# unibas-gravis/icp-proposal

Measured on AMD Instinct MI355X. Metric: ICP-proposal MH iterations/sec (femur GPMM r=50, ~50k-vtx target), higher is better.
Workload: dtype f64

## Files before the change

__graft_entry__.py:

```python
from __future__ import annotations

import importlib.util
import os
import subprocess
import sys

ROOT = os.path.dirname(os.path.abspath(__file__))
PKG_DIR = os.path.join(ROOT, "icp-proposal_amd")


def load_package():
    if "icp_proposal_amd" in sys.modules:
        return sys.modules["icp_proposal_amd"]
    spec = importlib.util.spec_from_file_location("icp_proposal_amd", os.path.join(PKG_DIR, "__init__.py"),
                                                  submodule_search_locations=[PKG_DIR])
    mod = importlib.util.module_from_spec(spec)
    sys.modules["icp_proposal_amd"] = mod
    spec.loader.exec_module(mod)
    return mod


def build() -> None:
    subprocess.run(["make", "-C", os.path.join(PKG_DIR, "csrc"), "-j4"], check=True)
    host_mk = os.path.join(PKG_DIR, "host", "Makefile")
    if os.path.exists(host_mk):
        subprocess.run(["make", "-C", os.path.join(PKG_DIR, "host")], check=True)
    subprocess.run(["make", "-C", os.path.join(ROOT, "oracle")], check=True)
    subprocess.run(["make", "-C", os.path.join(ROOT, "tests", "support")], check=True)
    pkg = load_package()
    pkg._native.lib()


def smoke() -> None:
    import numpy as np

    pkg = load_package()
    sys.path.insert(0, ROOT)
    from oracle import oracle as O

    model, target = pkg.data.load_femur_model_and_target(50)
    ctx = pkg.IcpContext(model, target, device=0)
    om, ot = O.OracleModel.from_model(model), O.OracleMesh(target.points, target.cells)
    r = model.rank
    rng = np.random.default_rng(7)
    theta = pkg.initial_parameters(model)
    theta[10:] = 0.3 * rng.normal(size=r)
    z = rng.normal(size=r)
    tp = pkg.data.decimated_point_subset(target, 2 * r)
    for direction, pp in ((pkg.ModelSampling, O.proposal_params(0.1, 10.0, 5.0, O.MODEL_SAMPLING, True, n_model_ids=2 * r)),
                          (pkg.TargetSampling, O.proposal_params(0.1, 10.0, 5.0, O.TARGET_SAMPLING, True, target_pts=tp))):
        prop = pkg.NonRigidIcpProposal(ctx, 0.1, 10.0, 5.0, 2 * r, direction, True, decimatedTargetPoints=tp)
        got, corr = prop.propose(theta, z, return_correspondences=True)
        want = O.propose(om, ot, pp, theta, z)
        post = O.icp_posterior(om, ot, pp, theta)
        assert np.array_equal(corr, np.where(post.keep == 1, post.corr_id, -1)), "correspondence indices differ"
        rel = np.abs(got - want).max() / np.abs(want[10:]).max()
        assert rel < 1e-5, f"proposed coefficients differ: {rel}"
        lt, lo = prop.logTransitionProbability(theta, got), O.log_transition(om, ot, pp, theta, want)
        assert abs(lt - lo) <= 1e-5 * abs(lo), (lt, lo)
        prop.close()
    ev = pkg.IndependentPointDistanceEvaluator(ctx, 0.0, 2.0, pkg.ModelToTargetEvaluation, 4 * r, decimatedTargetPoints=tp)
    ep = O.evaluator_params(O.EVAL_INDEPENDENT, O.MODEL_TO_TARGET, n_model_ids=4 * r, target_pts=tp, p0=0.0, p1=2.0)
    lv, (lvo, _) = ev.logValue(theta), O.evaluator_log_value(om, ot, ep, theta)
    assert abs(lv - lvo) <= 1e-9 * abs(lvo), (lv, lvo)
    ev.close()
    ctx.close()
    print("smoke ok: correspondence indices bit-exact, coefficients/logT/logValue within tolerance")


if __name__ == "__main__":
    build()
    if len(sys.argv) > 1 and sys.argv[1] == "smoke":
        smoke()
```

icp-proposal_amd/csrc/kernels_eigen.hip:

```cpp
#include <algorithm>
#include <atomic>
#include <cstdio>
#include <cstdlib>

#include "icp_kernels.hpp"
#include "icp_dense.hpp"

namespace icp {

#ifdef ICP_EIGEN_TIMING
__device__ long long g_eigen_stamps[64];
#define EIG_STAMP(i) do { if (threadIdx.x == 0) g_eigen_stamps[i] = __builtin_amdgcn_s_memrealtime(); } while (0)
#else
#define EIG_STAMP(i)
#endif
}
#include "icp_tridiag.hpp"
namespace icp {

namespace {

constexpr int kEigenMaxSweeps = 40;
#ifndef ICP_LOOSE_TAU
#define ICP_LOOSE_TAU 4e-6
// ... 100 lines not shown
      const double vkp = V[op], vkq = V[oq];
      V[op] = c * vkp - s * vkq;
      V[oq] = s * vkp + c * vkq;
    }
  };
  int converged = 0, n_sweeps = 0;
  for (int sweep = 0; sweep < 40 && !converged; ++sweep) {
    for (int rnd = 0; rnd < mm; ++rnd) {
      if (tid < half) {
        const int p = ra < rb ? ra : rb, q = ra < rb ? rb : ra;
        double c = 1.0, s = 0.0;
        if (q < r) {
          const double apq = A[p * lda + q], app = A[p * lda + p], aqq = A[q * lda + q];
          if (fabs(apq) > 1e-300 && apq * apq > 1e-36 * fabs(app * aqq)) {
            const double a = 0.5 * (aqq - app);
            const double h2 = fma(a, a, apq * apq);
            const double h = h2 * fast_rsqrt(h2);
            const double t = (a >= 0.0 ? apq : -apq) * fast_rcp(fabs(a) + h);
            c = fast_rsqrt(fma(t, t, 1.0));
            s = t * c;
          }
        }
        s_p[tid] = (short)p; s_q[tid] = (short)q; s_c[tid] = c; s_s[tid] = s;
        if (tid == 0) { rb = rb + 1 == mm ? 0 : rb + 1; }
        else { ra = ra + 1 == mm ? 0 : ra + 1; rb = rb + 1 == mm ? 0 : rb + 1; }
      }
      __syncthreads();
#pragma unroll
      for (int m = 0; m < kItems; ++m) {
        if (it_a[m] >= 0) {
          if (it_a[m] & 0x40000000) do_vpair(it_a[m] & 0x3FFFFFFF, it_b[m]);
          else do_block(it_a[m], it_b[m]);
        }
      }
      for (int w = tid + nt * kItems; w < n_items; w += nt) {
        if (w < n_blocks) {
          int P1 = 0, base = 0;
          while (base + (half - P1) <= w) { base += half - P1; ++P1; }
          do_block(P1, P1 + (w - base));
        } else {
          const int vi = w - n_blocks;
          do_vpair(vi / half, vi % half);
        }
      }
      __syncthreads();
    }
    double off = 0.0, dg = 0.0;
    for (int e = tid; e < r * r; e += nt) {
      const int i = e / r, j = e - i * r;
      const double v = A[(size_t)i * lda + j];
      if (i == j) dg = fma(v, v, dg);
      else off = fma(v, v, off);
    }
    off = block_sum(off, s_red);
    dg = block_sum(dg, s_red);
    converged = off <= 1e-26 * dg;
    n_sweeps = sweep + 1;
  }
  if (tid == 0) { status[0] = converged ? 0 : 2; status[-1] = n_sweeps; }
  for (int i = tid; i < r; i += nt) s_mu[i] = A[(size_t)i * lda + i];
  __syncthreads();
  for (int i = tid; i < r; i += nt) {
    int rank = 0;
    const double mi = s_mu[i];
    for (int j = 0; j < r; ++j) rank += (s_mu[j] < mi) || (s_mu[j] == mi && j < i);
    s_rank[i] = rank;
    int best = 0;
    double bv = fabs(V[i]);
    for (int k = 1; k < r; ++k) {
      const double a = fabs(V[(size_t)k * ldv + i]);
      if (a > bv) { bv = a; best = k; }
    }
    s_sgn[i] = V[(size_t)best * ldv + i] < 0.0 ? -1.0 : 1.0;
    Sout[rank] = 1.0 / mi;
  }
  __syncthreads();
  if (!v_in_lds) {
    for (int e = tid; e < r * r; e += nt) work[e] = V[e];
    __syncthreads();
    V = work;
  }
  for (int e = tid; e < r * r; e += nt) {
    const int k = e / r, i = e - k * r;
    const double v = V[(size_t)k * ldv + i] * s_sgn[i];
    Vout[(size_t)k * r + s_rank[i]] = v;
    Vtout[(size_t)s_rank[i] * r + k] = v;
  }
}


__device__ __forceinline__ int rr_dst(int pos, int m) {
  const int k = pos >> 1;
  if ((pos & 1) == 0) return k == 0 ? 0 : (k == m - 1 ? 2 * (m - 1) + 1 : 2 * (k + 1));
  return k == 0 ? 2 : 2 * (k - 1) + 1;
}
__device__ __forceinline__ int rr_src(int pos, int m) {
  const int k = pos >> 1;
  if ((pos & 1) == 0) return k == 0 ? 0 : (k == 1 ? 1 : 2 * (k - 1));
  return k == m - 1 ? 2 * (m - 1) : 2 * (k + 1) + 1;
}

struct Rot { double c, s; };

__device__ __forceinline__ Rot jacobi_rotation(double app, double apq, double aqq) {
  const double a = aqq - app, b = apq + apq, b2 = b * b;
  const bool rot = apq * apq > 1e-36 * fabs(app * aqq);
  const double h2 = fma(a, a, b2);
  const double h = h2 * __builtin_amdgcn_rsq(h2);
  const double u = h + fabs(a);
  const double w = fma(u, u, b2);
  const double y0 = __builtin_amdgcn_rsq(w);
  const double e = fma(-(0.5 * w) * y0, y0, 0.5);
  const double y = fma(y0, e * fma(1.5, e, 1.0), y0);
  Rot R;
  R.c = rot ? u * y : 1.0;
  R.s = rot ? (a >= 0.0 ? b : -b) * y : 0.0;
  return R;
}

struct B22 { double a00, a01, a10, a11; };

__device__ __forceinline__ B22 rot_block(B22 b, double c1, double s1, double c2, double s2) {
  const double t00 = fma(c1, b.a00, -(s1 * b.a10)), t01 = fma(c1, b.a01, -(s1 * b.a11));
  const double t10 = fma(s1, b.a00, c1 * b.a10), t11 = fma(s1, b.a01, c1 * b.a11);
  return B22{fma(c2, t00, -(s2 * t01)), fma(s2, t00, c2 * t01), fma(c2, t10, -(s2 * t11)), fma(s2, t10, c2 * t11)};
}
typedef double dbl2 __attribute__((ext_vector_type(2)));
__device__ __forceinline__ dbl2 lds2(const double* p) { return *(const dbl2*)p; }


constexpr int kPwRoundsMask = 0x3FFFF, kPwAbort = 1 << 18, kPwFinished = 1 << 19, kPwIdShift = 20, kPwIdMask = 0x7FF;
__device__ __forceinline__ void progress_publish(int* meta, int id, int rounds, int flags) {
  __hip_atomic_store(meta, (id << kPwIdShift) | flags | rounds, __ATOMIC_RELAXED, __HIP_MEMORY_SCOPE_AGENT);
}

__device__ __forceinline__ double wave_shr1_f64(double v) {
  const int lo = __builtin_amdgcn_update_dpp(__double2loint(v), __double2loint(v), 0x138, 0xf, 0xf, false);
  const int hi = __builtin_amdgcn_update_dpp(__double2hiint(v), __double2hiint(v), 0x138, 0xf, 0xf, false);
  return __hiloint2double(hi, lo);
}
__device__ __forceinline__ double wave_shl1_f64(double v) {
  const int lo = __builtin_amdgcn_update_dpp(__double2loint(v), __double2loint(v), 0x130, 0xf, 0xf, false);
  const int hi = __builtin_amdgcn_update_dpp(__double2hiint(v), __double2hiint(v), 0x130, 0xf, 0xf, false);
  return __hiloint2double(hi, lo);
}

constexpr int kReplayStageRounds = 64;
constexpr int kReplayWaves = 8;
constexpr int kReplayRows = 4 * kReplayWaves;
constexpr int kEigMetaCorr = 7;
constexpr int kEigMetaMu = 64;
constexpr int kEigMetaXchg = 128;

__device__ __forceinline__ void sc1_store(double* p, double v) { __hip_atomic_store(p, v, __ATOMIC_RELAXED, __HIP_MEMORY_SCOPE_AGENT); }
__device__ __forceinline__ double sc1_load(const double* p) { return __hip_atomic_load(p, __ATOMIC_RELAXED, __HIP_MEMORY_SCOPE_AGENT); }

__device__ void eigen_replay_consumer(int r, const double* Vwarm, const double* rotlog, int* meta, const double* xcorr ,
                                      double* Vout, double* Vtout, double* Sout, int launch_id, int me, int nb, int* done_word,
                                      int done_value) {
  __shared__ int s_pw;
  const int tid = threadIdx.x, lane = tid & 63, wave = tid >> 6;
  const int n2 = (r + 1) & ~1, m = n2 >> 1;
  double* s_log = s_dyn;
  const int kc = lane >> 5, q = lane & 31, ka = kReplayRows * me + 4 * wave + 2 * kc, kb = ka + 1;
  const bool carry = wave < kReplayWaves && kReplayRows * me + 4 * wave < r;
  const bool act = q < m && carry;
  const int qc = q < m ? q : 0;
  auto v0_at = [&](int k, int p) { return (k < r && p < r) ? (Vwarm ? Vwarm[(size_t)k * r + p] : (k == p ? 1.0 : 0.0)) : 0.0; };
  double a0 = act ? v0_at(ka, 2 * q) : 0.0, a1 = act ? v0_at(ka, 2 * q + 1) : 0.0;
  double b0 = act ? v0_at(kb, 2 * q) : 0.0, b1 = act ? v0_at(kb, 2 * q + 1) : 0.0;
  int done = 0;
  bool aborted = false;
  for (;;) {
    if (tid == 0) {
      int pw;
      for (;;) {
        pw = __hip_atomic_load(meta, __ATOMIC_RELAXED, __HIP_MEMORY_SCOPE_AGENT);
        if (((pw >> kPwIdShift) & kPwIdMask) == launch_id && ((pw & kPwRoundsMask) > done || (pw & (kPwAbort | kPwFinished)))) break;
        __builtin_amdgcn_s_sleep(2);
      }
      s_pw = pw;
#ifdef ICP_EIGEN_TIMING
      if (me == 0 && (pw & kPwFinished)) g_eigen_stamps[40] = __builtin_amdgcn_s_memrealtime();
#endif
    }
    __syncthreads();
    const int pw = s_pw;
    if (pw & kPwAbort) { aborted = true; break; }
    const int avail = pw & kPwRoundsMask;
    while (done < avail) {
      const int n = min(avail - done, kReplayStageRounds);
      for (int e = tid; e < 2 * n * m; e += blockDim.x) s_log[e] = sc1_load(rotlog + 2 * (size_t)done * m + e);
      __syncthreads();
      if (carry) {
        for (int rl = 0; rl < n; rl += 8) {
          dbl2 cs[8];
#pragma unroll
          for (int u = 0; u < 8; ++u) cs[u] = *(const dbl2*)&s_log[2 * (min(rl + u, n - 1) * m + qc)];
#pragma unroll
          for (int u = 0; u < 8; ++u) {
            if (rl + u < n) {
              const double fa = fma(cs[u].x, a0, cs[u].y * a1), ga = fma(-cs[u].y, a0, cs[u].x * a1);
              const double fb = fma(cs[u].x, b0, cs[u].y * b1), gb = fma(-cs[u].y, b0, cs[u].x * b1);
              const double ua = wave_shr1_f64(q == 0 ? ga : fa), da = wave_shl1_f64(ga);
              const double ub = wave_shr1_f64(q == 0 ? gb : fb), db = wave_shl1_f64(gb);
              a0 = q == 0 ? fa : ua; a1 = q == m - 1 ? fa : da;
              b0 = q == 0 ? fb : ub; b1 = q == m - 1 ? fb : db;
            }
          }
        }
      }
      __syncthreads();
      done += n;
    }
    if (pw & kPwFinished) break;
  }
#ifdef ICP_EIGEN_TIMING
  if (me == 0 && tid == 0) g_eigen_stamps[41] = __builtin_amdgcn_s_memrealtime();
#endif
  double* s_x = s_dyn;
  double* s_mu = s_dyn + 4096;
  int* s_rank = (int*)(s_dyn + 4096 + 64);
  double* s_bv = s_dyn + 4096 + 128;
  int* s_bk = (int*)(s_dyn + 4096 + 192);
  double* s_pv = s_dyn + 4096 + 256;
  int* s_pk = (int*)(s_dyn + 4096 + 256 + kReplayWaves * 64);
  double* xchg = (double*)meta + kEigMetaXchg;
  if (!aborted) {
    const int has_corr = __hip_atomic_load(meta + kEigMetaCorr, __ATOMIC_RELAXED, __HIP_MEMORY_SCOPE_AGENT);
    if (tid < n2) s_mu[tid] = sc1_load((const double*)meta + kEigMetaMu + tid);
    if (has_corr)
      for (int e = tid; e < n2 * n2; e += blockDim.x) s_x[e] = sc1_load(xcorr + e);
    __syncthreads();
    if (has_corr) {
      if (act) {
        *(dbl2*)&s_dyn[5632 + (4 * wave + 2 * kc) * 64 + 2 * q] = dbl2{a0, a1};
        *(dbl2*)&s_dyn[5632 + (4 * wave + 2 * kc + 1) * 64 + 2 * q] = dbl2{b0, b1};
      }
      __syncthreads();
      if (carry) {
        double ca0 = 0.0, ca1 = 0.0, cb0 = 0.0, cb1 = 0.0;
        const int ra = 5632 + (4 * wave + 2 * kc) * 64, rb = ra + 64;
        for (int i = 0; i < n2; i += 2) {
          const dbl2 va = *(const dbl2*)&s_dyn[ra + i], vb = *(const dbl2*)&s_dyn[rb + i];
          const dbl2 xe = *(const dbl2*)&s_dyn[i * n2 + 2 * qc], xo = *(const dbl2*)&s_dyn[(i + 1) * n2 + 2 * qc];
          ca0 = fma(va.x, xe.x, ca0); ca1 = fma(va.x, xe.y, ca1); cb0 = fma(vb.x, xe.x, cb0); cb1 = fma(vb.x, xe.y, cb1);
          ca0 = fma(va.y, xo.x, ca0); ca1 = fma(va.y, xo.y, ca1); cb0 = fma(vb.y, xo.x, cb0); cb1 = fma(vb.y, xo.y, cb1);
        }
        if (act) { a0 += ca0; a1 += ca1; b0 += cb0; b1 += cb1; }
      }
    }
    if (wave < kReplayWaves) {
      const bool va = act && ka < r, vb = act && kb < r;
      double m0 = va ? fabs(a0) : -1.0, m1 = va ? fabs(a1) : -1.0, c0 = a0, c1 = a1;
      int k0 = ka, k1 = ka;
      if (vb && fabs(b0) > m0) { m0 = fabs(b0); c0 = b0; k0 = kb; }
      if (vb && fabs(b1) > m1) { m1 = fabs(b1); c1 = b1; k1 = kb; }
      const double o0 = __shfl_xor(m0, 32, 64), o1 = __shfl_xor(m1, 32, 64), w0 = __shfl_xor(c0, 32, 64), w1 = __shfl_xor(c1, 32, 64);
      const int ok0 = __shfl_xor(k0, 32, 64), ok1 = __shfl_xor(k1, 32, 64);
      if (o0 > m0 || (o0 == m0 && ok0 < k0)) { m0 = o0; c0 = w0; k0 = ok0; }
      if (o1 > m1 || (o1 == m1 && ok1 < k1)) { m1 = o1; c1 = w1; k1 = ok1; }
      if (lane < 32 && q < m) {
        s_pv[wave * 64 + 2 * q] = m0 < 0.0 ? 0.0 : c0; s_pk[wave * 64 + 2 * q] = m0 < 0.0 ? 0x7fffffff : k0;
        s_pv[wave * 64 + 2 * q + 1] = m1 < 0.0 ? 0.0 : c1; s_pk[wave * 64 + 2 * q + 1] = m1 < 0.0 ? 0x7fffffff : k1;
      }
    }
    __syncthreads();
    if (tid < n2) {
      double bv = s_pv[tid];
      int bk = s_pk[tid];
      for (int w = 1; w < kReplayWaves; ++w) {
        const double v = s_pv[w * 64 + tid];
        const int kk = s_pk[w * 64 + tid];
        if (kk != 0x7fffffff && (bk == 0x7fffffff || fabs(v) > fabs(bv) || (fabs(v) == fabs(bv) && kk < bk))) { bv = v; bk = kk; }
      }
      s_bv[tid] = bv; s_bk[tid] = bk;
      if (nb > 1) { sc1_store(xchg + me * 128 + tid, bv); sc1_store(xchg + me * 128 + 64 + tid, (double)bk); }
      int rank = 0;
      const double mi = s_mu[tid];
      for (int j = 0; j < n2; ++j) rank += (s_mu[j] < mi) || (s_mu[j] == mi && j < tid);
      s_rank[tid] = rank;
      if (me == 0 && rank < r) sc1_store(Sout + rank, 1.0 / mi);
    }
    if (nb > 1) {
      asm volatile("s_waitcnt vmcnt(0)" ::: "memory");
      __syncthreads();
      const int o = 1 - me;
      if (tid == 0) {
        __hip_atomic_store(meta + 2 + me, launch_id, __ATOMIC_RELAXED, __HIP_MEMORY_SCOPE_AGENT);
        while (__hip_atomic_load(meta + 2 + o, __ATOMIC_RELAXED, __HIP_MEMORY_SCOPE_AGENT) != launch_id) __builtin_amdgcn_s_sleep(1);
      }
      __syncthreads();
      if (tid < n2) {
        const double v = sc1_load(xchg + o * 128 + tid);
        const int kk = (int)sc1_load(xchg + o * 128 + 64 + tid);
        double bv = s_bv[tid];
        const int bk = s_bk[tid];
        if (kk != 0x7fffffff && (bk == 0x7fffffff || fabs(v) > fabs(bv) || (fabs(v) == fabs(bv) && kk < bk))) bv = v;
        s_bv[tid] = bv;
      }
      if (tid == 0) __hip_atomic_store(meta + 2 + o, 0, __ATOMIC_RELAXED, __HIP_MEMORY_SCOPE_AGENT);
    }
    __syncthreads();
    if (act) {
      const int p0 = 2 * q, p1 = 2 * q + 1, r0 = s_rank[p0], r1 = s_rank[p1];
      const bool n0 = s_bv[p0] < 0.0, n1 = s_bv[p1] < 0.0;
      if (ka < r) {
        if (r0 < r) { const double v = n0 ? -a0 : a0; sc1_store(Vout + (size_t)ka * r + r0, v); sc1_store(Vtout + (size_t)r0 * r + ka, v); }
        if (r1 < r) { const double v = n1 ? -a1 : a1; sc1_store(Vout + (size_t)ka * r + r1, v); sc1_store(Vtout + (size_t)r1 * r + ka, v); }
      }
      if (kb < r) {
        if (r0 < r) { const double v = n0 ? -b0 : b0; sc1_store(Vout + (size_t)kb * r + r0, v); sc1_store(Vtout + (size_t)r0 * r + kb, v); }
        if (r1 < r) { const double v = n1 ? -b1 : b1; sc1_store(Vout + (size_t)kb * r + r1, v); sc1_store(Vtout + (size_t)r1 * r + kb, v); }
      }
    }
  }
#ifdef ICP_EIGEN_TIMING
  if (me == 0 && tid == 0) g_eigen_stamps[42] = __builtin_amdgcn_s_memrealtime();
#endif
  asm volatile("s_waitcnt vmcnt(0)" ::: "memory");
  __syncthreads();
  if (tid == 0) {
    if (nb == 1 || __hip_atomic_fetch_add(meta + 1, 1, __ATOMIC_RELAXED, __HIP_MEMORY_SCOPE_AGENT) == nb - 1) {
      __hip_atomic_store(meta + 1, 0, __ATOMIC_RELAXED, __HIP_MEMORY_SCOPE_AGENT);
      __hip_atomic_store(meta, 0, __ATOMIC_RELAXED, __HIP_MEMORY_SCOPE_AGENT);
      if (done_word) __hip_atomic_store(done_word, done_value, __ATOMIC_RELAXED, __HIP_MEMORY_SCOPE_AGENT);
    }
  }
}

constexpr int kRrLd = 66;
constexpr int kRrSzA = 64 * kRrLd;
constexpr int kRrSzC = 4 * 32;
constexpr int kRrOC = 0, kRrOA = 2 * kRrSzC, kRrOV = kRrOA + 2 * kRrSzA;
constexpr int kRrLogWave = 14;
constexpr int kRrPollWave = 13;
constexpr int kRrLogLag = 8;
template <int N> struct IntC { static constexpr int value = N; };

template <int CAP> struct EigenBatch {
  int n; EigenProblem p[CAP];
  __device__ __forceinline__ void announce() const {}
  __device__ __forceinline__ bool skipped(int) const { return false; }
};
struct EigenBatchMem {
  int n; const EigenProblem* p; int* arrive;
  const int* skip = nullptr;
  __device__ __forceinline__ void announce() const {
    if (arrive && threadIdx.x == 0) __hip_atomic_fetch_add(arrive, 1, __ATOMIC_RELAXED, __HIP_MEMORY_SCOPE_AGENT);
  }
  __device__ __forceinline__ bool skipped(int which) const { return skip != nullptr && skip[which] != 0; }
};
static_assert(sizeof(EigenBatch<2>) + 64 <= 4096, "the batch record must fit the kernel argument segment");

template <class Batch>
__global__ void __launch_bounds__(1024) k_posterior_eigen_rr(int r, const double* __restrict__ sqrt_lambda_launch, int ldk, int max_sweeps,
                                                              int no_corr , Batch batch) {
  batch.announce();
  const int per = 1 + (r + kReplayRows - 1) / kReplayRows;
  const int which = (int)blockIdx.x / per, local = (int)blockIdx.x - which * per;
  if (batch.skipped(which)) return;
  const EigenProblem pb = batch.p[which];
  const double* __restrict__ sqrt_lambda = pb.sqrt_lambda ? pb.sqrt_lambda : sqrt_lambda_launch;
  const double* __restrict__ M = pb.M;
  const double* Vwarm = pb.Vwarm;
  double* Vout = pb.Vout;
  double* Vtout = pb.Vtout;
  double* __restrict__ Sout = pb.Sout;
  int* __restrict__ status = pb.status;
  double* rotlog = pb.rotlog;
  int* meta = pb.meta;
  double* vpos = pb.vpos;
  const EigenSpec spec = pb.spec;
  const int launch_id = pb.launch_id;
  int* host_status = pb.host_status;
  if (Vwarm && !(Vwarm[0] == Vwarm[0])) Vwarm = nullptr;
  if (local != 0) {
    eigen_replay_consumer(r, Vwarm, rotlog, meta, vpos, Vout, Vtout, Sout, launch_id, local - 1, per - 1, pb.done_word, pb.done_value);
    return;
  }
  __shared__ double s_red[16], s_red2[16];
  __shared__ int s_cancel, s_bad[16];
  const int tid = threadIdx.x, nt = blockDim.x, lane = tid & 63, wave = tid >> 6;
  const int n2 = (r + 1) & ~1, m = n2 >> 1;
  constexpr int ld = kRrLd, szA = kRrSzA, szC = kRrSzC, oA = kRrOA, oV = kRrOV, oC = kRrOC;
  const int szV = n2 * ldk, oT = oV + szV;
#define LDS_A(b, i) s_dyn[oA + (b) * szA + (i)]
#define LDS_VT(i) s_dyn[oV + (i)]
#define LDS_T(i) s_dyn[oT + (i)]
#define LDS_C(b, i) s_dyn[oC + (b) * szC + (i)]
  EIG_STAMP(0);
  const bool is_poll = spec.cancel != nullptr && tid == 64 * kRrPollWave + 63;
  if (tid == 0) s_cancel = 0;
  for (int e = tid; e < szV; e += nt) LDS_VT(e) = 0.0;
  __syncthreads();
  const int nA = m * (m + 1) / 2, nbw = (nA + 63) >> 6;
  const int widx = (wave & 3) == 3 ? -1 : wave - (wave >> 2);
  const int bidx = (widx >= 0 && widx < nbw) ? widx * 64 + lane : nA;
  const bool is_blk = bidx < nA;
  int bI = 0, bJ = 0, b_rd = 0, w00 = 0, w01 = 0, w10 = 0, w11 = 0;
  if (is_blk) {
    int base = 0;
    while (base + (m - bI) <= bidx) { base += m - bI; ++bI; }
    bJ = bI + (bidx - base);
    b_rd = 2 * bI * ld + 2 * bJ;
    const int R0 = rr_dst(2 * bI, m), R1 = rr_dst(2 * bI + 1, m), C0 = rr_dst(2 * bJ, m), C1 = rr_dst(2 * bJ + 1, m);
    w00 = min(R0, C0) * ld + max(R0, C0); w01 = min(R0, C1) * ld + max(R0, C1);
    w10 = min(R1, C0) * ld + max(R1, C0); w11 = min(R1, C1) * ld + max(R1, C1);
  }
  const bool is_rot = wave == 3 && lane < m;
  int rp_dp = 0, rp_dq = 0, rp_ob = 0, rp_cp = 0, rp_cq = 0, rp_cl = 0, rp_ch = 0, rp_k = 0;
  if (wave == 3) {
    __builtin_amdgcn_s_setprio(3);
    rp_k = is_rot ? lane : 0;
    const int p = rr_src(2 * rp_k, m), q = rr_src(2 * rp_k + 1, m);
    const int ip = p >> 1, ap = p & 1, iq = q >> 1, aq = q & 1, lo = min(ip, iq), hi = max(ip, iq);
    const int ra = ip < iq ? ap : aq, ca = ip < iq ? aq : ap;
    rp_dp = 2 * ip * ld + 2 * ip; rp_dq = 2 * iq * ld + 2 * iq; rp_ob = 2 * lo * ld + 2 * hi;
    rp_cp = 4 * ip + 2 * ap; rp_cq = 4 * iq + 2 * aq; rp_cl = 4 * lo + 2 * ra; rp_ch = 4 * hi + 2 * ca;
  }
  for (int e = tid; e < r * r; e += nt) {
    const int i = e / r, j = e - i * r;
    LDS_VT(j * ldk + i) = Vwarm ? Vwarm[e] : (i == j ? 1.0 : 0.0);
  }
  EIG_STAMP(50);
  if (spec.ready) {
    if (is_poll) {
      const long long t0 = __builtin_amdgcn_s_memrealtime();
      for (;;) {
        if (__hip_atomic_load(spec.ready, __ATOMIC_ACQUIRE, __HIP_MEMORY_SCOPE_AGENT) - spec.ready_seq >= 0) break;
        if (__hip_atomic_load(spec.cancel, __ATOMIC_RELAXED, __HIP_MEMORY_SCOPE_SYSTEM) == spec.seq) { s_cancel = 1; break; }
        if (__builtin_amdgcn_s_memrealtime() - t0 > 500000) { s_cancel = 2; break; }
        __builtin_amdgcn_s_sleep(32);
      }
      if (spec.wait_ticks) atomicAdd((unsigned long long*)spec.wait_ticks, (unsigned long long)(__builtin_amdgcn_s_memrealtime() - t0));
    }
    __syncthreads();
    __builtin_amdgcn_fence(__ATOMIC_ACQUIRE, "agent");
  }
  EIG_STAMP(51);
  if (is_poll && !spec.ready && __hip_atomic_load(spec.cancel, __ATOMIC_RELAXED, __HIP_MEMORY_SCOPE_SYSTEM) == spec.seq) s_cancel = 1;
  if (spec.splits > 0) {
    for (int e = tid; e < n2 * n2; e += nt) {
      const int i = e / n2, j = e - i * n2;
      LDS_A(0, i * ld + j) = (i == j && i >= r) ? 1e300 : 0.0;
    }
    __syncthreads();
    const size_t nn = (size_t)(r + 1) * (r + 1);
    const int jp = tid & 31, j0 = 2 * jp;
    dbl2 acc[2] = {dbl2{0.0, 0.0}, dbl2{0.0, 0.0}};
    bool live[2];
    size_t off[2];
#pragma unroll
    for (int h = 0; h < 2; ++h) {
      const int i = (tid >> 5) + 32 * h;
      live[h] = i < r && j0 <= i;
      off[h] = live[h] ? (size_t)i * (r + 1) + j0 : 0;
    }
    const bool aligned = ((r + 1) & 1) == 0;
    int sp = 0;
    for (; sp + 8 <= spec.splits; sp += 8) {
      dbl2 p[8][2];
#pragma unroll
      for (int q8 = 0; q8 < 8; ++q8)
#pragma unroll
        for (int h = 0; h < 2; ++h) {
          const double* src = M + (size_t)(sp + q8) * nn + off[h];
          p[q8][h] = aligned ? *(const dbl2*)src : dbl2{src[0], src[1]};
        }
#pragma unroll
      for (int q8 = 0; q8 < 8; ++q8)
#pragma unroll
        for (int h = 0; h < 2; ++h) acc[h] += p[q8][h];
    }
    for (; sp < spec.splits; ++sp) {
#pragma unroll
      for (int h = 0; h < 2; ++h) {
        const double* src = M + (size_t)sp * nn + off[h];
        acc[h] += aligned ? *(const dbl2*)src : dbl2{src[0], src[1]};
      }
    }
#pragma unroll
    for (int h = 0; h < 2; ++h)
      if (live[h]) {
        const int i = (tid >> 5) + 32 * h;
        const double si = sqrt_lambda[i];
        double v0 = acc[h].x + (i == j0 ? 1.0 : 0.0);
        v0 = v0 / (si * sqrt_lambda[j0]);
        LDS_A(0, i * ld + j0) = v0; LDS_A(0, j0 * ld + i) = v0;
        if (j0 + 1 <= i) {
          double v1 = acc[h].y + (i == j0 + 1 ? 1.0 : 0.0);
          v1 = v1 / (si * sqrt_lambda[j0 + 1]);
          LDS_A(0, i * ld + j0 + 1) = v1; LDS_A(0, (j0 + 1) * ld + i) = v1;
        }
      }
  } else {
    for (int e = tid; e < n2 * n2; e += nt) {
      const int i = e / n2, j = e - i * n2;
      double v = i == j ? 1e300 : 0.0;
      if (i < r && j < r) v = 0.5 * (M[(size_t)i * r + j] + M[(size_t)j * r + i]) / (sqrt_lambda[i] * sqrt_lambda[j]);
      LDS_A(0, i * ld + j) = v;
    }
  }
  __syncthreads();
  if (s_cancel) {
    if (tid == 0) {
      progress_publish(meta, launch_id, 0, kPwAbort);
      if (s_cancel == 2) {
        if (host_status) __hip_atomic_store(host_status, kEigenGaveUp, __ATOMIC_RELAXED, __HIP_MEMORY_SCOPE_SYSTEM);
        Vout[0] = __builtin_nan("");
      }
    }
    return;
  }
  EIG_STAMP(1);
  if (Vwarm) {
    const int tI = wave >> 2, tJ = wave & 3, nT = (n2 + 15) >> 4, l15 = lane & 15, l4 = lane >> 4;
    {
      const int j = 16 * tI + l15, i = 16 * tJ + l15;
      const bool vj = j < r, vi = i < r;
      const int jc = vj ? j : 0, ic = vi ? i : 0;
      d4_t acc = {0.0, 0.0, 0.0, 0.0};
      if (tI < nT && tJ < nT) {
#pragma unroll
        for (int h = 0; h < 16; h += 8) {
        double av[8], bv[8];
#pragma unroll
        for (int st = 0; st < 8; ++st) {
          const int k = 4 * (h + st) + l4;
          const bool vk = k < r;
          const int kk = vk ? k : 0;
          const double a = LDS_VT(jc * ldk + kk), b = LDS_A(0, kk * ld + ic);
          av[st] = (vj && vk) ? a : 0.0; bv[st] = (vi && vk) ? b : 0.0;
        }
#pragma unroll
        for (int st = 0; st < 8; ++st)
          if (4 * (h + st) < n2) acc = __builtin_amdgcn_mfma_f64_16x16x4f64(av[st], bv[st], acc, 0, 0, 0);
        }
#pragma unroll
        for (int g = 0; g < 4; ++g) {
          const int row = 16 * tI + l4 + 4 * g;
          if (row < n2 && i < n2) LDS_T(row * ldk + i) = acc[g];
        }
      }
    }
    __syncthreads();
    {
      const int i = 16 * tI + l15, j = 16 * tJ + l15;
      const bool vi = i < r, vj = j < r;
      const int ic = vi ? i : 0, jc = vj ? j : 0;
      d4_t acc = {0.0, 0.0, 0.0, 0.0};
      if (tI <= tJ && tJ < nT) {
#pragma unroll
        for (int h = 0; h < 16; h += 8) {
        double av[8], bv[8];
#pragma unroll
        for (int st = 0; st < 8; ++st) {
          const int k = 4 * (h + st) + l4;
          const bool vk = k < r;
          const int kk = vk ? k : 0;
          const double a = LDS_VT(ic * ldk + kk), b = LDS_T(jc * ldk + kk);
          av[st] = (vi && vk) ? a : 0.0; bv[st] = (vj && vk) ? b : 0.0;
        }
#pragma unroll
        for (int st = 0; st < 8; ++st)
          if (4 * (h + st) < n2) acc = __builtin_amdgcn_mfma_f64_16x16x4f64(av[st], bv[st], acc, 0, 0, 0);
        }
#pragma unroll
        for (int g = 0; g < 4; ++g) {
          const int row = 16 * tI + l4 + 4 * g;
          if (row <= j && j < r) LDS_A(0, row * ld + j) = acc[g];
        }
      }
    }
    __syncthreads();
  }
  EIG_STAMP(2);

  if (wave == 3) {
    const int o = 2 * rp_k * ld + 2 * rp_k;
    const Rot R = jacobi_rotation(LDS_A(0, o), LDS_A(0, o + 1), LDS_A(0, o + ld + 1));
    if (is_rot) { LDS_C(0, 4 * rp_k) = R.c; LDS_C(0, 4 * rp_k + 1) = -R.s; LDS_C(0, 4 * rp_k + 2) = R.s; LDS_C(0, 4 * rp_k + 3) = R.c; }
  }
  const bool is_log = wave == kRrLogWave && lane < m;
  const size_t lstride = (size_t)2 * m;
  __syncthreads();
  EIG_STAMP(3);

  int n_rounds = 0, pub_floor = 0;
  auto round = [&](auto CUR) {
    constexpr int cur = decltype(CUR)::value;
    constexpr int ac = oA + cur * szA, an = oA + (cur ^ 1) * szA, cc = oC + cur * szC, cn = oC + (cur ^ 1) * szC;
    if (is_blk) {
      const dbl2 r0 = lds2(&s_dyn[ac + b_rd]), r1 = lds2(&s_dyn[ac + b_rd + ld]);
      const dbl2 c1 = lds2(&s_dyn[cc + 4 * bI]), c2 = lds2(&s_dyn[cc + 4 * bJ]);
      const bool dg = bI == bJ;
      const B22 n = rot_block(B22{r0.x, r0.y, dg ? r0.y : r1.x, r1.y}, c1.x, -c1.y, c2.x, -c2.y);
      s_dyn[an + w00] = n.a00; s_dyn[an + w01] = n.a01; s_dyn[an + w10] = n.a10; s_dyn[an + w11] = n.a11;
    } else if (wave == 3) {
      const dbl2 dp0 = lds2(&s_dyn[ac + rp_dp]), dp1 = lds2(&s_dyn[ac + rp_dp + ld]);
      const dbl2 dq0 = lds2(&s_dyn[ac + rp_dq]), dq1 = lds2(&s_dyn[ac + rp_dq + ld]);
      const dbl2 b0 = lds2(&s_dyn[ac + rp_ob]), b1 = lds2(&s_dyn[ac + rp_ob + ld]);
      const dbl2 kp = lds2(&s_dyn[cc + rp_cp]), kq = lds2(&s_dyn[cc + rp_cq]);
      const dbl2 kl = lds2(&s_dyn[cc + rp_cl]), kh = lds2(&s_dyn[cc + rp_ch]);
      __builtin_amdgcn_sched_barrier(0);
      const double app = fma(kp.x * kp.x, dp0.x, (kp.x * kp.y) * dp0.y) + fma(kp.y * kp.x, dp0.y, (kp.y * kp.y) * dp1.y);
      const double aqq = fma(kq.x * kq.x, dq0.x, (kq.x * kq.y) * dq0.y) + fma(kq.y * kq.x, dq0.y, (kq.y * kq.y) * dq1.y);
      const double apq = fma(kh.x * kl.x, b0.x, (kh.x * kl.y) * b1.x) + fma(kh.y * kl.x, b0.y, (kh.y * kl.y) * b1.y);
      const Rot R = jacobi_rotation(app, apq, aqq);
      if (is_rot) {
        *(dbl2*)&s_dyn[cn + 4 * rp_k] = dbl2{R.c, -R.s};
        *(dbl2*)&s_dyn[cn + 4 * rp_k + 2] = dbl2{R.s, R.c};
      }
    } else if (wave == kRrLogWave) {
      if (is_log) {
        const dbl2 k = lds2(&s_dyn[cc + 4 * lane]);
        const dbl2 w = fabs(k.y) >= 2e-17 ? k : dbl2{1.0, 0.0};
        double* dst = rotlog + (size_t)n_rounds * lstride + 2 * lane;
        sc1_store(dst, w.x); sc1_store(dst + 1, w.y);
      }
      if ((n_rounds & 3) == 3) {
        asm volatile("s_waitcnt vmcnt(%0)" :: "n"(2 * kRrLogLag + kRrLogLag / 4 - 1) : "memory");
        const int upto = n_rounds + 1 - kRrLogLag;
        if (lane == 0 && upto > pub_floor) __hip_atomic_store(meta, (launch_id << kPwIdShift) | upto, __ATOMIC_RELAXED, __HIP_MEMORY_SCOPE_AGENT);
      }
    }
    __syncthreads();
    ++n_rounds;
  };
  int converged = 0, n_sweeps = 0, in_sweep = 0, use_corr = 0;
  const int first_test = Vwarm ? 1 : 2;
  auto sweep_end = [&](int cur) -> bool {
    EIG_STAMP(4 + 2 * n_sweeps);
    in_sweep = 0;
    if (n_sweeps < first_test && n_sweeps + 1 < max_sweeps) {
      ++n_sweeps;
      EIG_STAMP(3 + 2 * n_sweeps);
      return s_cancel != 0;
    }
    if (wave == kRrLogWave) asm volatile("s_waitcnt vmcnt(0)" ::: "memory");
    pub_floor = n_rounds;
    double off = 0.0, dg = 0.0;
    bool bad = false;
    {
      const int i = tid >> 4, j0 = (tid & 15) << 2;
      if (i < n2 && j0 + 3 >= i && j0 < n2) {
        const dbl2 u = lds2(&LDS_A(cur, i * ld + j0)), w = lds2(&LDS_A(cur, i * ld + j0 + 2));
        const double dii = LDS_A(cur, i * ld + i);
        const double v[4] = {u.x, u.y, w.x, w.y};
#pragma unroll
        for (int c = 0; c < 4; ++c) {
          const int j = j0 + c;
          if (j < n2) {
            if (j == i) { if (v[c] < 1e299) dg = fma(v[c], v[c], dg); }
            else if (j > i) {
              off = fma(2.0 * v[c], v[c], off);
              bad = bad || fabs(v[c]) > kLooseTau * fabs(LDS_A(cur, j * ld + j) - dii);
            }
          }
        }
      }
    }
    for (int o = 32; o > 0; o >>= 1) { off += __shfl_xor(off, o, 64); dg += __shfl_xor(dg, o, 64); }
    const bool wave_bad = __any(bad);
    if (lane == 0) { s_red[wave] = off; s_red2[wave] = dg; s_bad[wave] = wave_bad ? 1 : 0; }
    __syncthreads();
    if (tid == 0) progress_publish(meta, launch_id, n_rounds, 0);
    off = 0.0; dg = 0.0;
    int any_bad = 0;
#pragma unroll
    for (int w = 0; w < 16; ++w) { off += s_red[w]; dg += s_red2[w]; any_bad |= s_bad[w]; }
    const int strict = off <= 1e-26 * dg;
    const int loose = !any_bad && off <= dg;
    converged = strict || (loose && !no_corr);
    use_corr = converged && !strict;
    if (tid == 0 && n_sweeps < 8) ((double*)(meta + 80))[n_sweeps] = off / dg;
    ++n_sweeps;
    EIG_STAMP(3 + 2 * n_sweeps);
    return converged || n_sweeps >= max_sweeps || s_cancel;
  };
  int cur = 0, polled = 0x80000000;
  const int poll_use = (n2 - 1) >> 2;
  if (max_sweeps > 0)
    for (;;) {
      if (is_poll && (in_sweep >> 1) == 0) polled = __hip_atomic_load(spec.cancel, __ATOMIC_RELAXED, __HIP_MEMORY_SCOPE_SYSTEM);
      if (is_poll && (in_sweep >> 1) == poll_use && polled == spec.seq) s_cancel = 1;
      round(IntC<0>{}); cur = 1;
      if (++in_sweep == n2 - 1 && sweep_end(cur)) break;
      round(IntC<1>{}); cur = 0;
      if (++in_sweep == n2 - 1 && sweep_end(cur)) break;
    }
  if (s_cancel && !converged) {
    if (tid == 0) progress_publish(meta, launch_id, n_rounds, kPwAbort);
    return;
  }
  if (tid == 0) {
    ++meta[100 + min(n_sweeps, 15)];
    status[0] = converged ? 0 : 2; status[-1] = n_sweeps;
    if (host_status) __hip_atomic_store(host_status, converged ? 0 : 2, __ATOMIC_RELAXED, __HIP_MEMORY_SCOPE_SYSTEM);
  }
  EIG_STAMP(62);
  double* xg = vpos;
  if (tid < n2) sc1_store((double*)meta + kEigMetaMu + tid, LDS_A(cur, tid * ld + tid));
  if (use_corr) {
    const int i = tid >> 4, j0 = (tid & 15) << 2;
    if (i < n2 && j0 + 3 >= i && j0 < n2) {
      const double dii = LDS_A(cur, i * ld + i);
#pragma unroll
      for (int c = 0; c < 4; ++c) {
        const int j = j0 + c;
        if (j < n2 && j >= i) {
          const double a = LDS_A(cur, i * ld + j);
          const double x = (j == i || a == 0.0) ? 0.0 : a / (LDS_A(cur, j * ld + j) - dii);
          sc1_store(xg + i * n2 + j, x);
          if (j != i) sc1_store(xg + j * n2 + i, -x);
        }
      }
    }
  }
  if (tid == 0) __hip_atomic_store(meta + kEigMetaCorr, use_corr, __ATOMIC_RELAXED, __HIP_MEMORY_SCOPE_AGENT);
  asm volatile("s_waitcnt vmcnt(0)" ::: "memory");
  __syncthreads();
  if (tid == 0) progress_publish(meta, launch_id, n_rounds, kPwFinished);
  EIG_STAMP(63);
#undef LDS_A
#undef LDS_VT
#undef LDS_T
#undef LDS_C
}

constexpr int kBigBlocksPerThread = 5;
constexpr int kBigMaxRank = 200;
constexpr int kBigSlabRows = 64;
constexpr int kBigStageRounds = 16;

__device__ __forceinline__ int big_idx(int i, int j, int n) {
  return i * (2 * n - i - 1) / 2 + (j - i - 1);
}
__device__ __forceinline__ void rr_init(int slot, int mm, int& ra, int& rb) {
  if (slot == 0) { ra = mm; rb = 0; }
  else { ra = slot % mm; rb = (mm - slot) % mm; }
}
__device__ __forceinline__ void rr_advance(int slot, int mm, int& ra, int& rb) {
  if (slot == 0) { rb = rb + 1 == mm ? 0 : rb + 1; }
  else { ra = ra + 1 == mm ? 0 : ra + 1; rb = rb + 1 == mm ? 0 : rb + 1; }
}

template <bool SQUARE>
__global__ void __launch_bounds__(1024) k_eigen_big(int r, const double* __restrict__ A0 , const double* __restrict__ Vwarm,
                                                     double* __restrict__ Vwork ,
                                                     double* __restrict__ mu_out, double* rotlog, double* xcorr , int* meta,
                                                     int max_sweeps, int no_corr, int launch_id, int* __restrict__ status,
                                                     const int* __restrict__ gate ) {
  if (gate && gate[0] != 2) return;
  const int tid = threadIdx.x, nt = blockDim.x;
  const int n = r, n2 = (r + 1) & ~1, half = n2 >> 1, mm = n2 - 1;
  __shared__ short s_p[128], s_q[128];
  __shared__ double s_red[16], s_red2[16];
  __shared__ int s_pw, s_bad[16];
  if (blockIdx.x != 0) {
    const int row0 = ((int)blockIdx.x - 1) * kBigSlabRows, rows = min(kBigSlabRows, r - row0);
    double* s_cs = s_dyn + kBigSlabRows * n;
    for (int e = tid; e < rows * n; e += nt) {
      const int k = e / n, p = e - k * n;
      s_dyn[e] = Vwarm ? Vwarm[(size_t)(row0 + k) * r + p] : (row0 + k == p ? 1.0 : 0.0);
    }
    int ra = 0, rb = 0;
    if (tid < half) rr_init(tid, mm, ra, rb);
    constexpr int kItems = 7;
    int itk[kItems], itP[kItems];
#pragma unroll
    for (int m = 0; m < kItems; ++m) {
      const int it = tid + m * nt;
      itk[m] = it < rows * half ? it / half : -1;
      itP[m] = it < rows * half ? it - itk[m] * half : 0;
    }
    int done = 0;
    for (;;) {
      if (tid == 0) {
        int pw;
        for (;;) {
          pw = __hip_atomic_load(meta, __ATOMIC_RELAXED, __HIP_MEMORY_SCOPE_AGENT);
          if (((pw >> kPwIdShift) & kPwIdMask) == launch_id && ((pw & kPwRoundsMask) > done || (pw & (kPwAbort | kPwFinished)))) break;
          __builtin_amdgcn_s_sleep(8);
        }
        s_pw = pw;
      }
      __syncthreads();
      const int pw = s_pw;
      const int avail = pw & kPwRoundsMask;
      while (done < avail) {
        const int nr = min(avail - done, kBigStageRounds);
        for (int e = tid; e < 2 * nr * half; e += nt) s_cs[e] = sc1_load(rotlog + 2 * (size_t)done * half + e);
        __syncthreads();
        for (int rl = 0; rl < nr; ++rl) {
          if (tid < half) {
            const int p = ra < rb ? ra : rb, q = ra < rb ? rb : ra;
            s_p[tid] = (short)p; s_q[tid] = (short)q;
            rr_advance(tid, mm, ra, rb);
          }
          __syncthreads();
#pragma unroll
          for (int m = 0; m < kItems; ++m) {
            if (itk[m] < 0) continue;
            const int k = itk[m], P = itP[m];
            const int p = s_p[P], q = s_q[P];
            if (q < r) {
              const dbl2 cs = *(const dbl2*)&s_cs[2 * (rl * half + P)];
              const double vp = s_dyn[k * n + p], vq = s_dyn[k * n + q];
              s_dyn[k * n + p] = fma(cs.x, vp, -(cs.y * vq));
              s_dyn[k * n + q] = fma(cs.y, vp, cs.x * vq);
            }
          }
          __syncthreads();
        }
        done += nr;
      }
      if (pw & (kPwFinished | kPwAbort)) break;
    }
    if (__hip_atomic_load(meta + 1, __ATOMIC_RELAXED, __HIP_MEMORY_SCOPE_AGENT) == launch_id) {
      for (int j0 = 0; j0 < n; j0 += 16) {
        __syncthreads();
        for (int e = tid; e < n * 16; e += nt) {
          const int i = e >> 4, j = j0 + (e & 15);
          s_cs[e] = j < n ? sc1_load(xcorr + (size_t)i * n + j) : 0.0;
        }
        __syncthreads();
        const int k = tid >> 4, j = j0 + (tid & 15);
        if (k < rows && j < n) {
          double acc = 0.0;
          for (int i = 0; i < n; ++i) acc = fma(s_dyn[k * n + i], s_cs[i * 16 + (tid & 15)], acc);
          Vwork[(size_t)(row0 + k) * r + j] = s_dyn[k * n + j] + acc;
        }
      }
    } else {
      for (int e = tid; e < rows * n; e += nt) Vwork[(size_t)row0 * r + e] = s_dyn[e];
    }
    return;
  }
  const int ld = SQUARE ? (n | 1) : 0;
  const int n_off = SQUARE ? n * ld : n * (n - 1) / 2;
  double* s_diag = s_dyn + n_off;
  double* s_cs = s_diag + n;
  auto at = [&](int i, int j) { return SQUARE ? i * ld + j : big_idx(i, j, n); };
  for (int e = tid; e < n * n; e += nt) {
// ... 549 lines not shown
```

Before: 11290.

## Poll eigen cancel flag every few rounds and add consumer wait timeouts

The Jacobi eigen kernel now polls the host cancel word on a fixed round cadence and breaks out mid-sweep, where before it checked only about once per sweep. An already-cancelled launch now returns before the setup work, and replay consumer blocks give up after a tick timeout instead of spinning forever. The aim is to stop speculative eigen solves sooner when they are cancelled and to avoid hangs, at the cost of extra polling and readfirstlane checks inside the rotation loop. A build step for a cancel-check tool is also added.

Result: faster. 12290, median of 6 (+8.9%).

```diff
diff --git a/__graft_entry__.py b/__graft_entry__.py
--- a/__graft_entry__.py
+++ b/__graft_entry__.py
@@ -27,6 +27,7 @@
         subprocess.run(["make", "-C", os.path.join(PKG_DIR, "host")], check=True)
     subprocess.run(["make", "-C", os.path.join(ROOT, "oracle")], check=True)
     subprocess.run(["make", "-C", os.path.join(ROOT, "tests", "support")], check=True)
+    subprocess.run(["make", "-C", os.path.join(ROOT, "tools"), "eigen_cancel_check"], check=True)
     pkg = load_package()
     pkg._native.lib()
 
diff --git a/icp-proposal_amd/csrc/kernels_eigen.hip b/icp-proposal_amd/csrc/kernels_eigen.hip
--- a/icp-proposal_amd/csrc/kernels_eigen.hip
+++ b/icp-proposal_amd/csrc/kernels_eigen.hip
@@ -276,12 +276,20 @@
 constexpr int kEigMetaMu = 64;
 constexpr int kEigMetaXchg = 128;
 
+constexpr unsigned long long kEigenWaitTicks = 500000;
+constexpr int kPwGaveUp = (int)0x80000000;
+
 __device__ __forceinline__ void sc1_store(double* p, double v) { __hip_atomic_store(p, v, __ATOMIC_RELAXED, __HIP_MEMORY_SCOPE_AGENT); }
 __device__ __forceinline__ double sc1_load(const double* p) { return __hip_atomic_load(p, __ATOMIC_RELAXED, __HIP_MEMORY_SCOPE_AGENT); }
 
+__device__ __forceinline__ void eigen_replay_gave_up(int* host_status, double* Vout) {
+  if (host_status) __hip_atomic_store(host_status, kEigenGaveUp, __ATOMIC_RELAXED, __HIP_MEMORY_SCOPE_SYSTEM);
+  Vout[0] = __builtin_nan("");
+}
+
 __device__ void eigen_replay_consumer(int r, const double* Vwarm, const double* rotlog, int* meta, const double* xcorr ,
                                       double* Vout, double* Vtout, double* Sout, int launch_id, int me, int nb, int* done_word,
-                                      int done_value) {
+                                      int done_value, int* host_status, bool awaits_input) {
   __shared__ int s_pw;
   const int tid = threadIdx.x, lane = tid & 63, wave = tid >> 6;
   const int n2 = (r + 1) & ~1, m = n2 >> 1;
@@ -297,10 +305,12 @@
   bool aborted = false;
   for (;;) {
     if (tid == 0) {
+      const unsigned long long t0 = __builtin_amdgcn_s_memrealtime(), limit = (awaits_input && done == 0) ? 2 * kEigenWaitTicks : kEigenWaitTicks;
       int pw;
       for (;;) {
         pw = __hip_atomic_load(meta, __ATOMIC_RELAXED, __HIP_MEMORY_SCOPE_AGENT);
         if (((pw >> kPwIdShift) & kPwIdMask) == launch_id && ((pw & kPwRoundsMask) > done || (pw & (kPwAbort | kPwFinished)))) break;
+        if (__builtin_amdgcn_s_memrealtime() - t0 > limit) { pw = kPwAbort | kPwGaveUp; break; }
         __builtin_amdgcn_s_sleep(2);
       }
       s_pw = pw;
@@ -310,7 +320,11 @@
     }
     __syncthreads();
     const int pw = s_pw;
-    if (pw & kPwAbort) { aborted = true; break; }
+    if (pw & kPwAbort) {
+      aborted = true;
+      if ((pw & kPwGaveUp) && tid == 0) eigen_replay_gave_up(host_status, Vout);
+      break;
+    }
     const int avail = pw & kPwRoundsMask;
     while (done < avail) {
       const int n = min(avail - done, kReplayStageRounds);
@@ -406,16 +420,23 @@
       s_rank[tid] = rank;
       if (me == 0 && rank < r) sc1_store(Sout + rank, 1.0 / mi);
     }
+    bool lost = false;
     if (nb > 1) {
       asm volatile("s_waitcnt vmcnt(0)" ::: "memory");
       __syncthreads();
       const int o = 1 - me;
       if (tid == 0) {
         __hip_atomic_store(meta + 2 + me, launch_id, __ATOMIC_RELAXED, __HIP_MEMORY_SCOPE_AGENT);
-        while (__hip_atomic_load(meta + 2 + o, __ATOMIC_RELAXED, __HIP_MEMORY_SCOPE_AGENT) != launch_id) __builtin_amdgcn_s_sleep(1);
+        const unsigned long long t0 = __builtin_amdgcn_s_memrealtime();
+        while (__hip_atomic_load(meta + 2 + o, __ATOMIC_RELAXED, __HIP_MEMORY_SCOPE_AGENT) != launch_id) {
+          if (__builtin_amdgcn_s_memrealtime() - t0 > kEigenWaitTicks) { s_pw = kPwAbort | kPwGaveUp; break; }
+          __builtin_amdgcn_s_sleep(1);
+        }
       }
       __syncthreads();
-      if (tid < n2) {
+      lost = (s_pw & kPwGaveUp) != 0;
+      if (lost && tid == 0) eigen_replay_gave_up(host_status, Vout);
+      if (tid < n2 && !lost) {
         const double v = sc1_load(xchg + o * 128 + tid);
         const int kk = (int)sc1_load(xchg + o * 128 + 64 + tid);
         double bv = s_bv[tid];
@@ -426,7 +447,7 @@
       if (tid == 0) __hip_atomic_store(meta + 2 + o, 0, __ATOMIC_RELAXED, __HIP_MEMORY_SCOPE_AGENT);
     }
     __syncthreads();
-    if (act) {
+    if (act && !lost) {
       const int p0 = 2 * q, p1 = 2 * q + 1, r0 = s_rank[p0], r1 = s_rank[p1];
       const bool n0 = s_bv[p0] < 0.0, n1 = s_bv[p1] < 0.0;
       if (ka < r) {
@@ -500,7 +521,8 @@
   int* host_status = pb.host_status;
   if (Vwarm && !(Vwarm[0] == Vwarm[0])) Vwarm = nullptr;
   if (local != 0) {
-    eigen_replay_consumer(r, Vwarm, rotlog, meta, vpos, Vout, Vtout, Sout, launch_id, local - 1, per - 1, pb.done_word, pb.done_value);
+    eigen_replay_consumer(r, Vwarm, rotlog, meta, vpos, Vout, Vtout, Sout, launch_id, local - 1, per - 1, pb.done_word, pb.done_value,
+                          host_status, spec.ready != nullptr);
     return;
   }
   __shared__ double s_red[16], s_red2[16];
@@ -516,6 +538,8 @@
   EIG_STAMP(0);
   const bool is_poll = spec.cancel != nullptr && tid == 64 * kRrPollWave + 63;
   if (tid == 0) s_cancel = 0;
+  int polled = 0x80000000;
+  if (is_poll) polled = __hip_atomic_load(spec.cancel, __ATOMIC_RELAXED, __HIP_MEMORY_SCOPE_SYSTEM);
   for (int e = tid; e < szV; e += nt) LDS_VT(e) = 0.0;
   __syncthreads();
   const int nA = m * (m + 1) / 2, nbw = (nA + 63) >> 6;
@@ -548,22 +572,34 @@
     LDS_VT(j * ldk + i) = Vwarm ? Vwarm[e] : (i == j ? 1.0 : 0.0);
   }
   EIG_STAMP(50);
-  if (spec.ready) {
+  if (spec.ready || spec.cancel) {
     if (is_poll) {
-      const long long t0 = __builtin_amdgcn_s_memrealtime();
-      for (;;) {
-        if (__hip_atomic_load(spec.ready, __ATOMIC_ACQUIRE, __HIP_MEMORY_SCOPE_AGENT) - spec.ready_seq >= 0) break;
-        if (__hip_atomic_load(spec.cancel, __ATOMIC_RELAXED, __HIP_MEMORY_SCOPE_SYSTEM) == spec.seq) { s_cancel = 1; break; }
-        if (__builtin_amdgcn_s_memrealtime() - t0 > 500000) { s_cancel = 2; break; }
-        __builtin_amdgcn_s_sleep(32);
-      }
-      if (spec.wait_ticks) atomicAdd((unsigned long long*)spec.wait_ticks, (unsigned long long)(__builtin_amdgcn_s_memrealtime() - t0));
-    }
-    __syncthreads();
-    __builtin_amdgcn_fence(__ATOMIC_ACQUIRE, "agent");
+      if (polled == spec.seq) s_cancel = 1;
+      else if (spec.ready) {
+        const unsigned long long t0 = __builtin_amdgcn_s_memrealtime();
+        for (;;) {
+          if (__hip_atomic_load(spec.ready, __ATOMIC_ACQUIRE, __HIP_MEMORY_SCOPE_AGENT) - spec.ready_seq >= 0) break;
+          if (__hip_atomic_load(spec.cancel, __ATOMIC_RELAXED, __HIP_MEMORY_SCOPE_SYSTEM) == spec.seq) { s_cancel = 1; break; }
+          if (__builtin_amdgcn_s_memrealtime() - t0 > kEigenWaitTicks) { s_cancel = 2; break; }
+          __builtin_amdgcn_s_sleep(32);
+        }
+        if (spec.wait_ticks) atomicAdd((unsigned long long*)spec.wait_ticks, (unsigned long long)(__builtin_amdgcn_s_memrealtime() - t0));
+      }
+    }
+    __syncthreads();
+    if (spec.ready) __builtin_amdgcn_fence(__ATOMIC_ACQUIRE, "agent");
+    if (s_cancel) {
+      if (tid == 0) {
+        progress_publish(meta, launch_id, 0, kPwAbort);
+        if (s_cancel == 2) {
+          if (host_status) __hip_atomic_store(host_status, kEigenGaveUp, __ATOMIC_RELAXED, __HIP_MEMORY_SCOPE_SYSTEM);
+          Vout[0] = __builtin_nan("");
+        }
+      }
+      return;
+    }
   }
   EIG_STAMP(51);
-  if (is_poll && !spec.ready && __hip_atomic_load(spec.cancel, __ATOMIC_RELAXED, __HIP_MEMORY_SCOPE_SYSTEM) == spec.seq) s_cancel = 1;
   if (spec.splits > 0) {
     for (int e = tid; e < n2 * n2; e += nt) {
       const int i = e / n2, j = e - i * n2;
@@ -627,16 +663,6 @@
     }
   }
   __syncthreads();
-  if (s_cancel) {
-    if (tid == 0) {
-      progress_publish(meta, launch_id, 0, kPwAbort);
-      if (s_cancel == 2) {
-        if (host_status) __hip_atomic_store(host_status, kEigenGaveUp, __ATOMIC_RELAXED, __HIP_MEMORY_SCOPE_SYSTEM);
-        Vout[0] = __builtin_nan("");
-      }
-    }
-    return;
-  }
   EIG_STAMP(1);
   if (Vwarm) {
     const int tI = wave >> 2, tJ = wave & 3, nT = (n2 + 15) >> 4, l15 = lane & 15, l4 = lane >> 4;
@@ -760,7 +786,7 @@
     if (n_sweeps < first_test && n_sweeps + 1 < max_sweeps) {
       ++n_sweeps;
       EIG_STAMP(3 + 2 * n_sweeps);
-      return s_cancel != 0;
+      return false;
     }
     if (wave == kRrLogWave) asm volatile("s_waitcnt vmcnt(0)" ::: "memory");
     pub_floor = n_rounds;
@@ -801,20 +827,31 @@
     if (tid == 0 && n_sweeps < 8) ((double*)(meta + 80))[n_sweeps] = off / dg;
     ++n_sweeps;
     EIG_STAMP(3 + 2 * n_sweeps);
-    return converged || n_sweeps >= max_sweeps || s_cancel;
+    return converged || n_sweeps >= max_sweeps;
   };
-  int cur = 0, polled = 0x80000000;
-  const int poll_use = (n2 - 1) >> 2;
+  const bool cancellable = spec.cancel != nullptr;
+  const bool poll_wave = cancellable && __builtin_amdgcn_readfirstlane(wave) == kRrPollWave;
+  bool cancelled = false;
+  int cur = 0, word = 0;
   if (max_sweeps > 0)
     for (;;) {
-      if (is_poll && (in_sweep >> 1) == 0) polled = __hip_atomic_load(spec.cancel, __ATOMIC_RELAXED, __HIP_MEMORY_SCOPE_SYSTEM);
-      if (is_poll && (in_sweep >> 1) == poll_use && polled == spec.seq) s_cancel = 1;
+      const int phase = n_rounds & 7;
+      if (poll_wave) {
+        if (phase == 0) word = __hip_atomic_load(spec.cancel, __ATOMIC_RELAXED, __HIP_MEMORY_SCOPE_SYSTEM);
+        if (phase == 4) {
+          asm volatile("" : "+v"(word));
+          if (lane == 63 && word == spec.seq) s_cancel = 1;
+        }
+      }
       round(IntC<0>{}); cur = 1;
-      if (++in_sweep == n2 - 1 && sweep_end(cur)) break;
+      if (cancellable && phase == 6) cancelled = __builtin_amdgcn_readfirstlane(s_cancel) != 0;
+      if (cancelled || (++in_sweep == n2 - 1 && sweep_end(cur))) break;
       round(IntC<1>{}); cur = 0;
       if (++in_sweep == n2 - 1 && sweep_end(cur)) break;
     }
-  if (s_cancel && !converged) {
+  if (cancelled) {
+    if (wave == kRrLogWave) asm volatile("s_waitcnt vmcnt(0)" ::: "memory");
+    __syncthreads();
     if (tid == 0) progress_publish(meta, launch_id, n_rounds, kPwAbort);
     return;
   }
```
